# oxfordcontrol/COSMO.jl

Measured on AMD Instinct MI355X. Metric: ADMM iterations/sec (fp64) at fixed (n,m,nnz,cone), higher is better.
Workload: dtype f64

## Files before the change

cosmo.jl_amd/csrc/api.hip:

```cpp
#include <stdarg.h>
#include <stdio.h>
#include <string.h>
#include <math.h>
#include <algorithm>
#include <chrono>
#include "internal.h"
#include "device_utils.h"
#include "value_maps.h"

int32_t cosmo_fail(cosmo_hip_handle* h, int32_t code, const char* fmt, ...) {
  char buf[1024];
  va_list ap;
  va_start(ap, fmt);
  vsnprintf(buf, sizeof buf, fmt, ap);
  va_end(ap);
  if (h) h->err = buf;
  return code;
}

template <class T>
static int32_t dalloc(cosmo_hip_handle* h, T** p, size_t count) {
  if (*p) { (void)hipFree(*p); *p = nullptr; }
  if (count == 0) count = 1;
  HIPCHK(h, hipMalloc((void**)p, count * sizeof(T)));
// ... 153 lines not shown
  p->check_termination = 25; p->check_infeasibility = 40; p->adaptive_rho = 1; p->adaptive_rho_interval = 40;
  p->adaptive_rho_fraction = 0.4; p->setup_time = 0.0;
  p->unscale_residuals = 1;
  p->obj_true = (double)NAN; p->obj_true_tol = 1e-3;
}

extern "C" int32_t cosmo_hip_create(cosmo_hip_handle** out, int32_t device_id) {
  if (!out) return COSMO_HIP_ERR_INVALID;
  *out = nullptr;
  int ndev = 0;
  if (hipGetDeviceCount(&ndev) != hipSuccess || ndev <= 0) return COSMO_HIP_ERR_HIP;
  if (device_id < 0 || device_id >= ndev) return COSMO_HIP_ERR_INVALID;
  cosmo_hip_handle* h = new cosmo_hip_handle();
  h->device = device_id;
  cosmo_hip_default_params(&h->prm);
  if (hipSetDevice(device_id) != hipSuccess || hipStreamCreate(&h->stream) != hipSuccess) { delete h; return COSMO_HIP_ERR_HIP; }
  if (hipMalloc((void**)&h->ctl, sizeof(Ctl)) != hipSuccess || hipHostMalloc((void**)&h->ctl_host, sizeof(Ctl)) != hipSuccess ||
      hipMalloc((void**)&h->partials, sizeof(real) * COSMO_NSLOTS_TOTAL * COSMO_MAX_PARTIALS) != hipSuccess) {
    delete h; return COSMO_HIP_ERR_HIP;
  }
  (void)hipMemset(h->ctl, 0, sizeof(Ctl));
  (void)hipMemset(h->partials, 0, sizeof(real) * COSMO_NSLOTS_TOTAL * COSMO_MAX_PARTIALS);
  memset(h->ctl_host, 0, sizeof(Ctl));
  (void)hipEventCreate(&h->ev_proj0);
  (void)hipEventCreate(&h->ev_proj1);
  *out = h;
  return COSMO_HIP_OK;
}

static void free_vectors(cosmo_hip_handle* h) {
// ... 571 lines not shown
  CHK(h2d(h, h->ctl, h->ctl_host, 1));
  h->host_iter = 0;
  h->have_iterates = true;
  h->fb_from = h->fb_recorded;
  return COSMO_HIP_OK;
}

static const int FB_LAG = 2;
static void feedback_reset(cosmo_hip_handle* h) { h->fb_from = h->fb_recorded; }
int32_t solve_budget(cosmo_hip_handle* h, int* budget_out) {
  const int R = cosmo_hip_handle::FB_RING;
  bool& used = h->fb_used[(h->host_solves + 1) % R];
  used = false;
  if (h->fb_mode == 1 && !h->fb_k) {
    if (const char* e = getenv("COSMO_HIP_BUDGET_FEEDBACK")) { if (atoi(e) == 0) h->fb_mode = 0; }
    if (h->fb_mode == 1 && hipHostMalloc((void**)&h->fb_k, sizeof(int) * cosmo_hip_handle::FB_RING) != hipSuccess) { (void)hipGetLastError(); h->fb_k = nullptr; h->fb_mode = 0; }
  }
  *budget_out = h->budget;
  if (h->fb_mode != 1 || h->profiling || h->exact_launches) return COSMO_HIP_OK;
  const long long j = h->fb_recorded - FB_LAG;
  const int wide = h->budget + h->budget / 16;
  if (j < h->fb_from || j < 0) { *budget_out = wide > 4096 ? 4096 : wide; return COSMO_HIP_OK; }
  HIPCHK(h, hipEventSynchronize(h->fb_ev[j % R]));
  int kmax = h->fb_k[j % R], kmin = kmax, nv = 1;
  for (long long i = j - 1; i >= h->fb_from && i > j - 4; --i) { const int v = h->fb_k[i % R]; kmax = std::max(kmax, v); kmin = std::min(kmin, v); nv += 1; }
  int b = (nv >= 3) ? kmax + (kmax - kmin) / 2 + kmax / 40 + 3 : kmax + (kmax * 15 + 99) / 100 + 6;
  if (b < 3) b = 3;
  if (b > 4096) b = 4096;
  used = true;
  h->cg_k_likely = kmax + 1;
  *budget_out = b;
  return COSMO_HIP_OK;
}
int32_t feedback_record(cosmo_hip_handle* h) {
  if (h->fb_mode != 1 || !h->fb_k) return COSMO_HIP_OK;
  const int R = cosmo_hip_handle::FB_RING;
  const int slot = (int)(h->fb_recorded % R);
  if (!h->fb_ev[slot]) HIPCHK(h, hipEventCreateWithFlags(&h->fb_ev[slot], hipEventDisableTiming));
  HIPCHK(h, hipMemcpyAsync(&h->fb_k[slot], &h->ctl->cg_k, sizeof(int), hipMemcpyDeviceToHost, h->stream));
  HIPCHK(h, hipEventRecord(h->fb_ev[slot], h->stream));
  h->fb_recorded += 1;
  return COSMO_HIP_OK;
}

static int32_t enqueue_solve_in_loop(cosmo_hip_handle* h) {
  CHK(enqueue_rhs(h, 1));
  CHK(kkt_enqueue_loop_solve(h));
  h->host_solves += 1;
  return COSMO_HIP_OK;
}

static bool inf_due(const cosmo_hip_handle* h, long long it) {
  const long long ci = h->prm.check_infeasibility;
  if (ci <= 0 || ci > (1LL << 40)) return false;
// ... 478 lines not shown
```

cosmo.jl_amd/csrc/internal.h:

```cpp
#pragma once
#include <hip/hip_runtime.h>
#include <stdint.h>
#include <string>
#include <vector>
#include "../../include/cosmo_hip.h"

typedef cosmo_hip_real real;
#ifdef COSMO_HIP_REAL_FLOAT
typedef float2 real2;
#define make_real2 make_float2
#define REAL_EPS 1.1920928955078125e-07f
#define REAL_MAX 3.402823466e+38f
#define REAL_IS_FLOAT 1
#else
typedef double2 real2;
#define make_real2 make_double2
#define REAL_EPS 2.220446049250313e-16
#define REAL_MAX 1.7976931348623157e308
#define REAL_IS_FLOAT 0
#endif
#define R(x) ((real)(x))

#define COSMO_BS 256
#define COSMO_NNZ_PER_BLOCK 2048
// ... 195 lines not shown
  real *w = nullptr, *w_prev = nullptr, *s = nullptr, *mu = nullptr, *s_tl = nullptr;
  real *ls_x = nullptr, *ls_s = nullptr, *x_tl = nullptr, *nu = nullptr;
  real *rhs = nullptr, *r = nullptr, *u = nullptr, *c = nullptr, *tmp_m = nullptr, *y2 = nullptr;
  real *mr = nullptr;
  real* partials = nullptr;
  Ctl* ctl = nullptr;
  Ctl* ctl_host = nullptr;
  real* io = nullptr;
  cosmo_hip_params prm;
  long long host_iter = 0;
  long long host_solves = 0;
  int budget = 12;
  long long stalls = 0;
  static const int FB_RING = 64;
  int* fb_k = nullptr;
  hipEvent_t fb_ev[FB_RING] = {};
  long long fb_recorded = 0;
  long long fb_from = 0;
  int fb_mode = 1;
  long long fb_stalls = 0;
  bool fb_used[FB_RING] = {};
  int cg_k_likely = 0x7fffffff;
  long long spmv_calls[3] = {0, 0, 0};
  bool profiling = false;
  bool exact_launches = false;
  std::vector<hipEvent_t> ev_pool;
  std::vector<std::pair<int, int>> ev_open;
  size_t ev_used = 0;
  double kc_seconds[COSMO_HIP_NUM_KERNEL_CLASSES] = {0};
  long long kc_launches[COSMO_HIP_NUM_KERNEL_CLASSES] = {0};
// ... 24 lines not shown
    int32_t rc__ = (call);                \
    if (rc__ != COSMO_HIP_OK) return rc__; \
  } while (0)

void build_row_blocks(const std::vector<int>& rowptr, int nrows, std::vector<int>& rb, int tile_override);
int32_t upload_csr(cosmo_hip_handle* h, const HostCsr& M, CsrDev& D, int split_col, int tile_override = 0);
void free_csr(CsrDev& D);
void prof_begin(cosmo_hip_handle* h, int kc);
void prof_end(cosmo_hip_handle* h);
int32_t prof_collect(cosmo_hip_handle* h);
int32_t sync_ctl(cosmo_hip_handle* h);
int32_t rebuild_cone_plans(cosmo_hip_handle* h);
int32_t reclassify_after_scaling(cosmo_hip_handle* h);
int32_t solve_budget(cosmo_hip_handle* h, int* budget_out);
int32_t feedback_record(cosmo_hip_handle* h);

int32_t build_op_split(cosmo_hip_handle* h, bool any_a, bool fold, int factor_min, long long factor_fill_min);
int32_t refresh_op_split(cosmo_hip_handle* h);
void free_op_split(cosmo_hip_handle* h);

int32_t kkt_configure(cosmo_hip_handle* h, bool force_split);
void kkt_free(cosmo_hip_handle* h);
int32_t kkt_update_rho(cosmo_hip_handle* h);
int32_t kkt_enqueue_refresh(cosmo_hip_handle* h);
int32_t kkt_enqueue_start(cosmo_hip_handle* h, int guard, real tol_k);
int32_t kkt_enqueue_iterations(cosmo_hip_handle* h, int guard, int k_begin, int count);
int32_t kkt_enqueue_loop_solve(cosmo_hip_handle* h);
int32_t kkt_solve_now(cosmo_hip_handle* h);
int32_t kkt_resume(cosmo_hip_handle* h, int extra);
bool kkt_krylov_model(const cosmo_hip_handle* h, double* bytes, int* launches);
// ... 122 lines not shown
```

cosmo.jl_amd/csrc/kernels.hip:

```cpp
#include "device_utils.h"

__global__ __launch_bounds__(COSMO_BS) void k_spmv_plain(CsrView M, const real* __restrict__ x, real* __restrict__ y) {
  __shared__ real lds[COSMO_NNZ_PER_BLOCK];
  __shared__ real red[COSMO_BS / 64];
  for (int b = blockIdx.x; b < M.nb; b += gridDim.x) {
    csr_stream_tile(M, x, x, tile_of_block(b, M.nb, M.xcd_affine), lds, red, [&](int r, real s1, real s2) { y[r] = s1 + s2; });
  }
}

__device__ __forceinline__ real project_simple(real x, uint32_t meta, const real* __restrict__ bl,
                                                 const real* __restrict__ bu) {
  const uint32_t kind = meta & 3u;
  if (kind == 0u) return x;
  if (kind == 1u) return 0.0;
  if (kind == 2u) {
    return (x != x) ? x : ((x > R(0.0)) ? x : R(0.0));
  }
  const uint32_t j = meta >> 2;
  const real l = bl[j], u = bu[j];
  return (x < l) ? l : ((x > u) ? u : x);
}

__global__ __launch_bounds__(COSMO_BS) void k_z(const Ctl* __restrict__ ctl, int guard, long long n, long long m,
                                                const real* __restrict__ w, real* __restrict__ w_prev,
// ... 322 lines not shown
    acc += ri * ri;
  }
  acc = block_sum(acc, red);
  if constexpr (PC) accz = block_sum(accz, red);
  if (threadIdx.x == 0) {
    part_rr[blockIdx.x] = acc;
    if constexpr (PC) part_rz[blockIdx.x] = accz;
    if (blockIdx.x == 0) ctl->cg_k = k + 1;
  }
}

__global__ __launch_bounds__(COSMO_BS) void k_tail(Ctl* __restrict__ ctl, int loop_mode, CsrView A, long long n, long long m,
                                                   real alpha, const real* __restrict__ x_tl,
                                                   const real* __restrict__ ls_s, const real* __restrict__ rho,
                                                   const real* __restrict__ s, real* __restrict__ nu,
                                                   real* __restrict__ s_tl, real* __restrict__ w, int nblk_rows) {
  if (loop_mode) {
    if (ctl->halt) return;
    if (!ctl->cg_done) {
      if (blockIdx.x == 0 && threadIdx.x == 0) { ctl->stalled = 1; ctl->halt = 1; }
      return;
    }
  }
  __shared__ real lds[COSMO_NNZ_PER_BLOCK];
  __shared__ real red[COSMO_BS / 64];
  if ((int)blockIdx.x < nblk_rows) {
    for (int k = blockIdx.x; k < A.nb; k += nblk_rows) {
      csr_stream_tile(A, x_tl, x_tl, k, lds, red, [&](int row, real s1, real s2) {
        const real ax = s1 + s2;
        const real rh = rho[row];
        const real nv = (ax - ls_s[row]) * rh;
        nu[row] = nv;
        if (loop_mode) {
          const real sv = s[row];
          const real wv = w[n + row];
          const real st = (R(2.0) * sv - wv) - nv / rh;
          s_tl[row] = st;
          w[n + row] = wv + alpha * (st - sv);
        }
      });
    }
  } else if (loop_mode) {
    const long long nb2 = gridDim.x - nblk_rows;
    for (long long i = (long long)(blockIdx.x - nblk_rows) * COSMO_BS + threadIdx.x; i < n; i += nb2 * COSMO_BS) {
      const real wv = w[i];
      w[i] = wv + alpha * (x_tl[i] - wv);
    }
    if ((int)blockIdx.x == nblk_rows && threadIdx.x == 0) {
      const int k = ctl->cg_k;
      ctl->iter += 1;
      ctl->solves += 1;
      ctl->kkt_iters_total += k;
      if (k > ctl->cg_k_max) ctl->cg_k_max = k;
    }
  }
}

__global__ void k_count_solve(Ctl* __restrict__ ctl) {
  const int k = ctl->cg_k;
  ctl->solves += 1;
  ctl->kkt_iters_total += k;
  if (k > ctl->cg_k_max) ctl->cg_k_max = k;
}

__global__ __launch_bounds__(COSMO_BS) void k_chk_prim(const Ctl* __restrict__ ctl, int guard, CsrView A, long long n,
                                                       const real* __restrict__ w_prev, const real* __restrict__ s,
                                                       const real* __restrict__ b, const real* __restrict__ rho,
                                                       const real* __restrict__ Einv, real* __restrict__ mu,
// ... 383 lines not shown
  return COSMO_HIP_OK;
}

int32_t enqueue_y2_only(cosmo_hip_handle* h) {
  hipLaunchKernelGGL(k_y2_only, dim3(ew_grid(h->m > 0 ? h->m : 1)), dim3(COSMO_BS), 0, h->stream, h->ctl, h->m, h->ls_s,
                     h->rho, h->y2);
  HIPCHK(h, hipGetLastError());
  return COSMO_HIP_OK;
}

int32_t enqueue_tail(cosmo_hip_handle* h, int loop_mode) {
  const int gr = h->A.grid > 0 ? h->A.grid : 1;
  const int gx = loop_mode ? ew_grid(h->n) : 0;
  prof_begin(h, KC_TAIL);
  hipLaunchKernelGGL(k_tail, dim3(gr + gx), dim3(COSMO_BS), 0, h->stream, h->ctl, loop_mode, view_of(h->A), h->n, h->m,
                     h->prm.alpha, h->x_tl, h->ls_s, h->rho, h->s, h->nu, h->s_tl, h->w, gr);
  prof_end(h);
  h->spmv_calls[0] += 1;
  HIPCHK(h, hipGetLastError());
  return COSMO_HIP_OK;
}

int32_t enqueue_count_solve(cosmo_hip_handle* h) {
  hipLaunchKernelGGL(k_count_solve, dim3(1), dim3(1), 0, h->stream, h->ctl);
  HIPCHK(h, hipGetLastError());
  return COSMO_HIP_OK;
}

int32_t enqueue_clear_stall(cosmo_hip_handle* h) {
  hipLaunchKernelGGL(k_ctl_clear_stall, dim3(1), dim3(1), 0, h->stream, h->ctl);
  HIPCHK(h, hipGetLastError());
// ... 125 lines not shown
```

cosmo.jl_amd/csrc/polar_tiles.h:

```cpp
#pragma once
#include <algorithm>
#include <vector>

constexpr int kPolarXcds = 8;
constexpr int kPolarPanelK = 16, kPolarStreamKTile = 96;

struct PolarCone {
  int idx;
  int off, d, kind;
  int ts;
  int sk;
  int skg, skc;
  int ld;
  long long woff;
};

struct BatchCone { long long woff; int off, d, kind, ld, idx, ts; };

struct QTile { int cone, ti, tj, pad; };

struct alignas(32) RTile { int cone; int i0, j0; int ext; int ld, d; long long woff; };

struct alignas(16) RPair { int cone; int i0, j0, i1, j1; int ext0, ext1; int ld, d; int pad; long long woff; };

// ... 16 lines not shown
struct PolarBatchPlan {
  std::vector<BatchCone> cones;
  long long work = 0;
  std::vector<QTile> qtiles;
  int nbtiles = 0, nbtiles96 = 0;
  std::vector<RTile> rtiles;
  std::vector<RTile> items;
  std::vector<RPair> pairs;
  int xoff[kPolarXcds + 1] = {};
  std::vector<int> cone_nt;
  int df_ntiles = 0;
  double flops_performed = 0.0, flops_useful = 0.0;
};
const char* polar_plan_batch(const std::vector<PolarBatchIn>& in, const PolarTileOpts& o, PolarBatchPlan& out);

long long polar_tile_cost(int d, int ext);

struct LiftDepth {
  int k, streak, patience;
  bool fail(int cap) {
    const bool up = k < cap;
    if (up) k += 1;
    streak = 0;
    patience = std::min(96, 2 * patience);
    return up;
  }
  bool pass(int floor) {
    if (++streak < patience || k <= floor) return false;
    k -= 1; streak = 0;
    return true;
// ... 3 lines not shown
```

cosmo.jl_amd/csrc/psd_polar.hip:

```cpp
#include "psd_internal.h"
#include "polar_tiles.h"
#include <math.h>
#include <stdlib.h>
#include <string.h>
#include <algorithm>
#include <mutex>

#define PK 16
#ifndef POLAR_PREFETCH_DEPTH
#define POLAR_PREFETCH_DEPTH 2
#endif
#define PLD 80
static_assert(PK == kPolarPanelK, "the planner's k panel");
static_assert(sizeof(QTile) == sizeof(int4), "the quadrant list is uploaded as the kernels' int4 array");

struct SkSync { unsigned ticket; unsigned timeout; unsigned pad[14]; unsigned flag[1]; };
struct PolarDev {
  int gate;
  int rounds;
  int verified;
  int unverified;
  int projections;
  int pad[3];
  real err_last, err_max;
// ... 26 lines not shown
  PolarDev* dev = nullptr;
  PolarDev seen;
  long long launches[4] = {0, 0, 0, 0};
  int streamk = 0;
  real* sk_scratch = nullptr;
  SkSync* sk_sync = nullptr;
  int sk_gmax = 0;
  unsigned sk_base = 0, sk_epoch = 0;
  int products_last_large = 0, products_last_batch = 0;
  std::vector<BatchCone> bcones;
  BatchCone* d_bcones = nullptr;
  int4* d_btiles = nullptr;
  int nbtiles = 0, nbtiles96 = 0;
  int speculate = 0;
  int* gate_host = nullptr;
  int batch_wave = 0;
  int batch_ragged = 1;
  void* d_rtiles = nullptr;
  int nrtiles = 0;
  int dataflow = 0;
  void* d_df_tiles = nullptr;
  int* d_df_cone_nt = nullptr;
  unsigned* d_df_sync = nullptr;
  int df_xoff[9] = {0, 0, 0, 0, 0, 0, 0, 0, 0};
  int df_grid = 0;
  int df_pair = 3;
  int df_ntiles = 0;
  long long df_launches = 0, df_timed = 0;
  int df_nprod = 0;
  double df_seconds = 0.0;
// ... 1147 lines not shown
__global__ __launch_bounds__(COSMO_BS) void k_bpolar_scale(const Ctl* __restrict__ ctl, int guard, const BatchCone* __restrict__ cones,
                                                           const real* __restrict__ parts, real* __restrict__ W, real* __restrict__ bnrm,
                                                           const int* __restrict__ ubuf) {
  if (guard && ctl->halt) return;
  const BatchCone cn = cones[blockIdx.y];
  real nf2 = 0.0;
  for (int k = 0; k < BPX; ++k) nf2 += parts[(size_t)blockIdx.y * 2 * BPX + k];
  const real nf = sqrt(nf2);
  const real inv = (nf > R(0.0)) ? R(2.0) / nf : R(0.0);
  if (blockIdx.x == 0 && threadIdx.x == 0) bnrm[blockIdx.y] = nf;
  const long long n2 = (long long)cn.ld * cn.ld;
  const real* X = W + cn.woff;
  real* U = W + cn.woff + (ubuf ? ubuf[blockIdx.y] : 1) * n2;
  for (long long i = (long long)blockIdx.x * COSMO_BS + threadIdx.x; i < n2; i += (long long)gridDim.x * COSMO_BS) U[i] = X[i] * inv;
}
__global__ __launch_bounds__(COSMO_BS) void k_bpolar_finish(const Ctl* __restrict__ ctl, int guard, const BatchCone* __restrict__ cones,
                                                            real* __restrict__ W, int iu, real* __restrict__ s, real* __restrict__ parts) {
  if (guard && ctl->halt) return;
  __shared__ real red[COSMO_BS / 64];
  const BatchCone cn = cones[blockIdx.y];
  const long long n2 = (long long)cn.ld * cn.ld;
  const real* X = W + cn.woff;
  const real* U = W + cn.woff + iu * n2;
  const real* H = W + cn.woff + 3 * n2;
  real* x = s + cn.off;
  const int d = cn.d, ld = cn.ld;
  real tr = 0.0;
  for (int j = blockIdx.x; j < d; j += gridDim.x) {
    for (int i = threadIdx.x; i <= j; i += COSMO_BS) {
      const long long o = (long long)j * ld + i;
      const real v = (X[o] + H[o]) / R(2.0);
      polar_write(x, cn.kind, d, i, j, v);
      const real u = U[o];
      tr += (i == j) ? (u + u * u) : R(2.0) * u * u;
    }
  }
  tr = block_sum(tr, red);
  if (threadIdx.x == 0) parts[(size_t)blockIdx.y * 2 * BPX + BPX + blockIdx.x] = tr;
}
__global__ void k_bpolar_rank(const Ctl* __restrict__ ctl, int guard, int n, const BatchCone* __restrict__ cones, const real* __restrict__ parts,
                              int* __restrict__ rank) {
  if (guard && ctl->halt) return;
  const int c = blockIdx.x * blockDim.x + threadIdx.x;
  if (c >= n) return;
  real tr = 0.0;
  for (int k = 0; k < BPX; ++k) tr += parts[(size_t)c * 2 * BPX + BPX + k];
  rank[cones[c].idx] = (int)llround(tr / (cones[c].kind == COSMO_HIP_PSD_TRIANGLE_COMPLEX ? R(4.0) : R(2.0)));
}

__global__ __launch_bounds__(COSMO_BS) void k_bpolar_sumsq(const Ctl* __restrict__ ctl, int guard, const int* __restrict__ gate, const BatchCone* __restrict__ cones,
                                                           const real* __restrict__ W, int ig, real* __restrict__ vparts) {
  if (guard && ctl->halt) return;
  if (gate && !gate[blockIdx.y]) return;
  __shared__ real red[COSMO_BS / 64];
  const BatchCone cn = cones[blockIdx.y];
  const long long n2 = (long long)cn.ld * cn.ld;
  const real* G = W + cn.woff + ig * n2;
  real acc = 0.0;
  for (long long i = (long long)blockIdx.x * COSMO_BS + threadIdx.x; i < n2; i += (long long)gridDim.x * COSMO_BS) { const real v = G[i]; acc += v * v; }
  acc = block_sum(acc, red);
  if (threadIdx.x == 0) vparts[(size_t)blockIdx.y * BPX + blockIdx.x] = acc;
}
__global__ __launch_bounds__(COSMO_BS) void k_bpolar_decide(const Ctl* __restrict__ ctl, int guard, PolarDev* __restrict__ pd, int* __restrict__ bgate, int round,
                                                            int last, int n, const BatchCone* __restrict__ cones, const real* __restrict__ vparts,
                                                            const real* __restrict__ bnrm, real tol_factor) {
  if (guard && ctl->halt) return;
  if (round > 0 && !pd->gate) return;
  __shared__ real red[COSMO_BS / 64];
  real emax = 0.0, nfail = 0.0, nchk = 0.0;
  for (int c = threadIdx.x; c < n; c += COSMO_BS) {
    if (round > 0 && !bgate[c]) continue;
    real g2 = 0.0;
    for (int k = 0; k < BPX; ++k) g2 += vparts[(size_t)c * BPX + k];
    const real nf = bnrm[c];
    const real err = (nf > R(0.0)) ? R(0.5) * sqrt(g2) / nf : R(0.0);
    const bool ok = !(err > tol_factor * cones[c].d * PSD_EPS);
    bgate[c] = (!ok && !last) ? 1 : 0;
    nchk += 1.0;
    if (!ok) nfail += 1.0;
    emax = (err > emax || err != err) ? err : emax;
  }
  emax = block_max(emax, red);
  nfail = block_sum(nfail, red);
  nchk = block_sum(nchk, red);
  if (threadIdx.x != 0) return;
  pd->err_last = emax;
  if (emax > pd->err_max || emax != emax) pd->err_max = emax;
  if (round == 0) pd->projections += 1; else pd->rounds += 1;
  if (nfail == R(0.0)) { pd->verified += 1; pd->gate = 0; }
  else if (last) { pd->unverified += 1; pd->gate = 0; }
  else pd->gate = 1;
  (void)nchk;
}

}

void polar_plan_destroy(cosmo_hip_handle* h) {
  PolarPlan* q = static_cast<PolarPlan*>(h->psd_polar);
  if (!q) return;
  if (q->W) (void)hipFree(q->W);
  if (q->parts) (void)hipFree(q->parts);
  if (q->nrm) (void)hipFree(q->nrm);
  if (q->gate_host) (void)hipHostFree(q->gate_host);
  if (q->sk_scratch) (void)hipFree(q->sk_scratch);
  if (q->sk_sync) (void)hipFree(q->sk_sync);
  if (q->d_bcones) (void)hipFree(q->d_bcones);
  if (q->d_btiles) (void)hipFree(q->d_btiles);
  if (q->d_rtiles) (void)hipFree(q->d_rtiles);
  if (q->d_rtiles_rep) (void)hipFree(q->d_rtiles_rep);
  if (q->rep_host) (void)hipHostFree(q->rep_host);
  free(q->h_rtiles);
  if (q->BW) (void)hipFree(q->BW);
  if (q->bparts) (void)hipFree(q->bparts);
  if (q->bnrm) (void)hipFree(q->bnrm);
  if (q->bgate) (void)hipFree(q->bgate);
  if (q->d_lgate) (void)hipFree(q->d_lgate);
  if (q->d_ubuf) (void)hipFree(q->d_ubuf);
  if (q->bgate_host) (void)hipHostFree(q->bgate_host);
// ... 1 lines not shown
  if (q->d_df_cone_nt) (void)hipFree(q->d_df_cone_nt);
  if (q->d_df_sync) (void)hipFree(q->d_df_sync);
  if (q->df_ev[0]) { (void)hipEventDestroy(q->df_ev[0]); (void)hipEventDestroy(q->df_ev[1]); }
  if (q->dev) (void)hipFree(q->dev);
  delete q;
  h->psd_polar = nullptr;
}

bool polar_enabled(const cosmo_hip_handle* h) { return h->psd_polar != nullptr; }

struct PolarKnobs {
  int large_jacobi = -1, k_lift = -1, adapt = 0, compact_repair = 1, rescale = 1, speculate = -1, rounds = -1, patience = 3;
  int streamk = 0, ts = 0, sk = 0;
  long long skg = 0;
  int ts96 = 0, wave = 0, flat = 0, ragged = 1, paired = -1, sort = 1, dataflow = -1, dataflow_grid = -1, occ = -1;
};

static PolarKnobs polar_read_knobs() {
  PolarKnobs k;
  auto flag = [](const char* name, int dflt) { const char* e = getenv(name); return e ? (atoi(e) ? 1 : 0) : dflt; };
  auto within = [](const char* name, int lo, int hi, int dflt) { const char* e = getenv(name); const int v = e ? atoi(e) : dflt; return (v >= lo && v <= hi) ? v : dflt; };
  if (const char* e = getenv("COSMO_HIP_PSD_LARGE")) k.large_jacobi = (e[0] == 'j') ? 1 : 0;
  if (const char* e = getenv("COSMO_HIP_POLAR_KLIFT")) k.k_lift = std::min(40, std::max(0, atoi(e)));
  k.adapt = flag("COSMO_HIP_POLAR_ADAPT", k.adapt);
  if (const char* e = getenv("COSMO_HIP_POLAR_PATIENCE")) k.patience = std::max(1, atoi(e));
  k.compact_repair = flag("COSMO_HIP_POLAR_COMPACT_REPAIR", k.compact_repair);
  k.rescale = flag("COSMO_HIP_POLAR_RESCALE", k.rescale);
  k.speculate = flag("COSMO_HIP_POLAR_SPECULATE", k.speculate);
  if (const char* e = getenv("COSMO_HIP_POLAR_ROUNDS")) k.rounds = std::min(8, std::max(0, atoi(e)));
  k.streamk = flag("COSMO_HIP_POLAR_STREAMK", k.streamk);
  if (const char* e = getenv("COSMO_HIP_POLAR_TS")) k.ts = atoi(e);
  if (const char* e = getenv("COSMO_HIP_POLAR_SK")) k.sk = atoi(e);
  if (const char* e = getenv("COSMO_HIP_POLAR_SKG")) k.skg = atoll(e);
  k.ts96 = flag("COSMO_HIP_POLAR_BATCH_TS96", k.ts96);
  k.wave = flag("COSMO_HIP_POLAR_BATCH_WAVE", k.wave);
  k.flat = getenv("COSMO_HIP_POLAR_BATCH_FLAT") ? 1 : 0;
  k.ragged = flag("COSMO_HIP_POLAR_BATCH_RAGGED", k.ragged);
  k.sort = flag("COSMO_HIP_POLAR_BATCH_SORT", k.sort);
  k.occ = within("COSMO_HIP_POLAR_BATCH_OCC", 3, 4, k.occ);
  k.paired = within("COSMO_HIP_POLAR_PAIRED", 0, 3, k.paired);
  k.dataflow = flag("COSMO_HIP_POLAR_DATAFLOW", k.dataflow);
  k.dataflow_grid = within("COSMO_HIP_POLAR_DATAFLOW_GRID", 8, 8192, k.dataflow_grid);
  return k;
}

static void polar_set_func_attributes(const PolarPlan* q) {
  if (q->bcones.empty()) return;
  if (q->batch_ragged) {
    (void)hipFuncSetAttribute((const void*)k_polar_dataflow<4>, hipFuncAttributeMaxDynamicSharedMemorySize, GemmCfg<64>::SMEM);
    (void)hipFuncSetAttribute((const void*)k_polar_dataflow_pair<4>, hipFuncAttributeMaxDynamicSharedMemorySize, DF_PAIR_SMEM);
    (void)hipFuncSetAttribute((const void*)k_symm_gemm_batch_r<0, 3>, hipFuncAttributeMaxDynamicSharedMemorySize, GemmCfg<64>::SMEM);
    (void)hipFuncSetAttribute((const void*)k_symm_gemm_batch_r<1, 3>, hipFuncAttributeMaxDynamicSharedMemorySize, GemmCfg<64>::SMEM);
    (void)hipFuncSetAttribute((const void*)k_symm_gemm_batch_r<0, 4>, hipFuncAttributeMaxDynamicSharedMemorySize, GemmCfg<64>::SMEM);
    (void)hipFuncSetAttribute((const void*)k_symm_gemm_batch_r<1, 4>, hipFuncAttributeMaxDynamicSharedMemorySize, GemmCfg<64>::SMEM);
  }
  (void)hipFuncSetAttribute((const void*)k_symm_gemm_batch<0, 3, 64>, hipFuncAttributeMaxDynamicSharedMemorySize, GemmCfg<64>::SMEM);
  (void)hipFuncSetAttribute((const void*)k_symm_gemm_batch<1, 3, 64>, hipFuncAttributeMaxDynamicSharedMemorySize, GemmCfg<64>::SMEM);
// ... 24 lines not shown
  PolarPlan* q = new PolarPlan();
  h->psd_polar = q;
  q->klift_forced = k.k_lift >= 0;
  if (q->klift_forced) q->k_lift = k.k_lift;
  q->adapt = k.adapt; q->compact_repair = k.compact_repair; q->rescale = k.rescale; q->streamk = k.streamk;
  q->batch_ts96 = k.ts96; q->batch_wave = k.wave;
  q->speculate = k.speculate >= 0 ? k.speculate : (large_list.size() > 2 ? 1 : 0);
  if (k.rounds >= 0) q->max_rounds = k.rounds;
  q->batch_ragged = (k.ragged && !k.ts96 && !k.wave) ? 1 : 0;
  if (k.paired >= 0) q->df_pair = k.paired;
  PolarTileOpts o;
  o.ts96 = k.ts96; o.flat = k.flat; o.ragged = q->batch_ragged; o.pair = q->df_pair; o.sort = k.sort;
  o.streamk = k.streamk; o.ts = k.ts; o.sk = k.sk; o.skg = k.skg;
  HIPCHK(h, hipHostMalloc((void**)&q->gate_host, 8 * sizeof(int), hipHostMallocDefault));
  for (int i = 0; i < 8; ++i) q->gate_host[i] = 0;
  HIPCHK(h, hipMalloc((void**)&q->dev, sizeof(PolarDev)));
  HIPCHK(h, hipMemset(q->dev, 0, sizeof(PolarDev)));
  memset(&q->seen, 0, sizeof(PolarDev));
  if (!large_list.empty()) {
    long long woff = 0;
    for (int idx : large_list) {
      const PsdConeDev& c = p->cones[idx];
      PolarCone pc;
      pc.idx = idx; pc.off = c.off; pc.d = c.d; pc.kind = c.kind;
      polar_plan_large(o, pc);
      q->sk_gmax = std::max(q->sk_gmax, pc.skg);
      pc.woff = woff;
      woff += 4LL * pc.ld * pc.ld;
      q->cones.push_back(pc);
    }
// ... 100 lines not shown
    kmax = 0;
    for (int c = 0; c < n; ++c) kmax = std::max(kmax, q->bdepth[c].k);
    if (q->lgate_kmax != kmax) {
      std::vector<int> lg((size_t)std::max(kmax, 1) * n, 0), ub((size_t)n, 1);
      for (int c = 0; c < n; ++c) {
        const int t0 = kmax - q->bdepth[c].k;
        for (int t = t0; t < kmax; ++t) lg[(size_t)t * n + c] = 1;
        ub[(size_t)c] = (t0 & 1) ? 2 : 1;
      }
      HIPCHK(h, hipMemcpyAsync(q->d_lgate, lg.data(), sizeof(int) * lg.size(), hipMemcpyHostToDevice, st));
      HIPCHK(h, hipMemcpyAsync(q->d_ubuf, ub.data(), sizeof(int) * ub.size(), hipMemcpyHostToDevice, st));
      HIPCHK(h, hipStreamSynchronize(st));
      q->lgate_kmax = kmax;
    }
  }
  hipLaunchKernelGGL(k_bpolar_populate, dim3(BPX, n), dim3(COSMO_BS), 0, st, h->ctl, guard, q->d_bcones, s, q->BW, q->bparts);
  hipLaunchKernelGGL(k_bpolar_scale, dim3(BPX, n), dim3(COSMO_BS), 0, st, h->ctl, guard, q->d_bcones, q->bparts, q->BW, q->bnrm, adapt ? (const int*)q->d_ubuf : (const int*)nullptr);
  int iu = 1, iy = 2, products = 0;
  DfArgs dfa;
  bool df = q->dataflow && q->batch_ragged && q->nrtiles > 0 && !adapt && !h->profiling && 3 * (kmax + POLAR_NFIN) + 2 <= DF_MAX_PROD;
  dfa.nprod = 0;
  auto product = [&](int epi, const int* gate, int ia, int ib, int icin, int ic, real alpha, real beta) {
    if (df) { DfProd& pr = dfa.prod[dfa.nprod++]; pr.ia = ia; pr.ib = ib; pr.icin = icin; pr.ic = ic; pr.epi = epi; pr.pad = 0; pr.alpha = alpha; pr.beta = beta; return; }
    if (epi) launch_bgemm<1>(q, st, h->ctl, guard, gate, ia, ib, icin, ic, alpha, beta);
    else launch_bgemm<0>(q, st, h->ctl, guard, gate, ia, ib, icin, ic, alpha, beta);
  };
  auto flush_dataflow = [&]() -> int32_t {
    if (!df) return COSMO_HIP_OK;
    for (int x = 0; x < 9; ++x) dfa.xoff[x] = q->df_xoff[x];
    HIPCHK(h, hipMemsetAsync(q->d_df_sync, 0, sizeof(unsigned) * (DF_SYNC_DONE + q->bcones.size()), st));
    if (!q->df_ev[0]) { HIPCHK(h, hipEventCreate(&q->df_ev[0])); HIPCHK(h, hipEventCreate(&q->df_ev[1])); }
    if (q->df_ev_pending && hipEventQuery(q->df_ev[1]) == hipSuccess) {
      float ms = 0.f;
      if (hipEventElapsedTime(&ms, q->df_ev[0], q->df_ev[1]) == hipSuccess) { q->df_seconds += 1e-3 * (double)ms; q->df_timed += 1; }
      q->df_ev_pending = 0;
    }
    (void)hipGetLastError();
    const bool timed = !q->df_ev_pending;
    if (timed) HIPCHK(h, hipEventRecord(q->df_ev[0], st));
    if (q->df_pair)
      hipLaunchKernelGGL((k_polar_dataflow_pair<4>), dim3(q->df_grid), dim3(512), DF_PAIR_SMEM, st, h->ctl, guard, (const RPair*)q->d_df_tiles, (const int*)q->d_df_cone_nt,
                         q->d_df_sync, q->BW, dfa);
    else
      hipLaunchKernelGGL((k_polar_dataflow<4>), dim3(q->df_grid), dim3(256), GemmCfg<64>::SMEM, st, h->ctl, guard, (const RTile*)q->d_df_tiles, (const int*)q->d_df_cone_nt,
                         q->d_df_sync, q->BW, dfa);
// ... 3 lines not shown
    return COSMO_HIP_OK;
  };
  auto step = [&](const real* co, const int* gate) {
    product(0, gate, iu, iu, iu, iy, 1.0, 0.0);
    product(1, gate, iy, iy, iy, 3, co[2], co[1]);
    product(1, gate, iu, 3, iu, iy, 1.0, co[0]);
    std::swap(iu, iy);
    products += 3; q->launches[3] += 3;
  };
  auto verify = [&](int round, const int* gate) -> int32_t {
    product(0, gate, iu, 0, 0, 3, 1.0, 0.0);
    product(1, gate, iu, 3, 0, iy, 1.0, -1.0);
    CHK(flush_dataflow());
    hipLaunchKernelGGL(k_bpolar_sumsq, dim3(BPX, n), dim3(COSMO_BS), 0, st, h->ctl, guard, gate, q->d_bcones, q->BW, iy, vparts);
    hipLaunchKernelGGL(k_bpolar_decide, dim3(1), dim3(COSMO_BS), 0, st, h->ctl, guard, q->dev, q->bgate, round, round == q->max_rounds ? 1 : 0, n, q->d_bcones,
                       vparts, q->bnrm, q->tol_factor);
    products += 2; q->launches[3] += 2;
    return COSMO_HIP_OK;
  };
  for (int t = 0; t < kmax; ++t) step(kPolarLift, adapt ? (const int*)(q->d_lgate + (size_t)t * n) : (const int*)nullptr);
  for (int t = 0; t < POLAR_NFIN; ++t) step(kPolarFinish[t], nullptr);
  CHK(verify(0, nullptr));
  q->products_last_batch = products;
  { double wsum = 0.0, w3 = 0.0;
    for (int c = 0; c < n; ++c) { const double d3 = (double)q->bcones[c].d * q->bcones[c].d * q->bcones[c].d; w3 += d3; wsum += d3 * (3.0 * ((adapt ? q->bdepth[c].k : kmax) + POLAR_NFIN) + 2.0); }
    q->wprod_last = w3 > 0.0 ? wsum / w3 : 0.0; }
  for (int r = 1; r <= q->max_rounds; ++r) {
    if (!q->speculate) {
      HIPCHK(h, hipMemcpyAsync(q->gate_host, &q->dev->gate, (adapt && r == 1 ? 5 : 1) * sizeof(int), hipMemcpyDeviceToHost, st));
      if (r == 1 && q->bgate_host) HIPCHK(h, hipMemcpyAsync(q->bgate_host, q->bgate, sizeof(int) * (size_t)n, hipMemcpyDeviceToHost, st));
      HIPCHK(h, hipStreamSynchronize(st));
      if (adapt && r == 1 && q->gate_host[4] != q->seen_proj_batch) {
        q->seen_proj_batch = q->gate_host[4];
        q->depth_proj += 1;
        bool changed = false;
        for (int c = 0; c < n; ++c) {
          if (*q->gate_host && q->bgate_host[c]) { q->depth_fail += 1; if (q->bdepth[c].fail(POLAR_LIFT_CAP)) changed = true; }
          else if (q->bdepth[c].pass(0)) { q->depth_down += 1; changed = true; }
        }
        if (changed) q->lgate_kmax = -1;
      }
      if (!*q->gate_host) break;
// ... 4 lines not shown
        const RTile* all = (const RTile*)q->h_rtiles; RTile* dst = (RTile*)q->rep_host;
        int cnt = 0;
        for (int t = 0; t < q->nrtiles; ++t) if (all[t].cone >= 0 && q->bgate_host[all[t].cone]) dst[cnt++] = all[t];
        if (cnt > 0) {
          HIPCHK(h, hipMemcpyAsync(q->d_rtiles_rep, dst, sizeof(RTile) * (size_t)cnt, hipMemcpyHostToDevice, st));
          q->nrep = cnt; q->repair_trains += 1;
        }
        if (adapt) rlift = 1;
      }
    }
    for (int t = 0; t < rlift; ++t) step(kPolarLift, q->bgate);
    for (int t = 0; t < POLAR_NFIN; ++t) step(kPolarFinish[t], q->bgate);
    CHK(verify(r, q->bgate));
  }
  q->nrep = 0;
  hipLaunchKernelGGL(k_bpolar_finish, dim3(BPX, n), dim3(COSMO_BS), 0, st, h->ctl, guard, q->d_bcones, q->BW, iu, s, q->bparts);
  hipLaunchKernelGGL(k_bpolar_rank, dim3((n + 63) / 64), dim3(64), 0, st, h->ctl, guard, n, q->d_bcones, q->bparts, p->rank);
  HIPCHK(h, hipGetLastError());
  return COSMO_HIP_OK;
}

int32_t polar_enqueue_project(cosmo_hip_handle* h, real* s, int guard) {
  PolarPlan* q = static_cast<PolarPlan*>(h->psd_polar);
  PsdPlan* p = h->psd;
  hipStream_t st = h->stream;
  for (size_t ci = 0; ci < q->cones.size(); ++ci) {
    const PolarCone& cn = q->cones[ci];
    const long long n2 = (long long)cn.ld * cn.ld;
    real* X = q->W + cn.woff;
    real* U = X + n2;
    real* Y = U + n2;
    real* T = Y + n2;
// ... 249 lines not shown
```

Before: 377.4.

## Use mapped host memory for feedback and polar gates, speculatively launch finish kernels

```diff
diff --git a/cosmo.jl_amd/csrc/api.hip b/cosmo.jl_amd/csrc/api.hip
--- a/cosmo.jl_amd/csrc/api.hip
+++ b/cosmo.jl_amd/csrc/api.hip
@@ -191,6 +191,7 @@
   cosmo_hip_handle* h = new cosmo_hip_handle();
   h->device = device_id;
   cosmo_hip_default_params(&h->prm);
+  if (const char* e = getenv("COSMO_HIP_STEP_PASSES")) h->step_passes = atoi(e) ? 1 : 0;
   if (hipSetDevice(device_id) != hipSuccess || hipStreamCreate(&h->stream) != hipSuccess) { delete h; return COSMO_HIP_ERR_HIP; }
   if (hipMalloc((void**)&h->ctl, sizeof(Ctl)) != hipSuccess || hipHostMalloc((void**)&h->ctl_host, sizeof(Ctl)) != hipSuccess ||
       hipMalloc((void**)&h->partials, sizeof(real) * COSMO_NSLOTS_TOTAL * COSMO_MAX_PARTIALS) != hipSuccess) {
@@ -792,7 +793,12 @@
   used = false;
   if (h->fb_mode == 1 && !h->fb_k) {
     if (const char* e = getenv("COSMO_HIP_BUDGET_FEEDBACK")) { if (atoi(e) == 0) h->fb_mode = 0; }
-    if (h->fb_mode == 1 && hipHostMalloc((void**)&h->fb_k, sizeof(int) * cosmo_hip_handle::FB_RING) != hipSuccess) { (void)hipGetLastError(); h->fb_k = nullptr; h->fb_mode = 0; }
+    const bool direct = h->step_passes && !h->row_shard;
+    if (h->fb_mode == 1 && hipHostMalloc((void**)&h->fb_k, sizeof(int) * cosmo_hip_handle::FB_RING, direct ? hipHostMallocMapped | hipHostMallocCoherent : hipHostMallocDefault) != hipSuccess) { (void)hipGetLastError(); h->fb_k = nullptr; h->fb_mode = 0; }
+    if (h->fb_k && direct) {
+      for (int i = 0; i < cosmo_hip_handle::FB_RING; ++i) h->fb_k[i] = 0;
+      HIPCHK(h, hipHostGetDevicePointer((void**)&h->fb_k_dev, h->fb_k, 0));
+    }
   }
   *budget_out = h->budget;
   if (h->fb_mode != 1 || h->profiling || h->exact_launches) return COSMO_HIP_OK;
@@ -810,12 +816,16 @@
   *budget_out = b;
   return COSMO_HIP_OK;
 }
+int* feedback_slot(const cosmo_hip_handle* h) {
+  if (h->fb_mode != 1 || !h->fb_k_dev || h->row_shard || h->route == KKT_MINRES_FULL || h->route == KKT_MINRES_REDUCED) return nullptr;
+  return h->fb_k_dev + h->fb_recorded % cosmo_hip_handle::FB_RING;
+}
 int32_t feedback_record(cosmo_hip_handle* h) {
   if (h->fb_mode != 1 || !h->fb_k) return COSMO_HIP_OK;
   const int R = cosmo_hip_handle::FB_RING;
   const int slot = (int)(h->fb_recorded % R);
   if (!h->fb_ev[slot]) HIPCHK(h, hipEventCreateWithFlags(&h->fb_ev[slot], hipEventDisableTiming));
-  HIPCHK(h, hipMemcpyAsync(&h->fb_k[slot], &h->ctl->cg_k, sizeof(int), hipMemcpyDeviceToHost, h->stream));
+  if (!feedback_slot(h)) HIPCHK(h, hipMemcpyAsync(&h->fb_k[slot], &h->ctl->cg_k, sizeof(int), hipMemcpyDeviceToHost, h->stream));
   HIPCHK(h, hipEventRecord(h->fb_ev[slot], h->stream));
   h->fb_recorded += 1;
   return COSMO_HIP_OK;
diff --git a/cosmo.jl_amd/csrc/internal.h b/cosmo.jl_amd/csrc/internal.h
--- a/cosmo.jl_amd/csrc/internal.h
+++ b/cosmo.jl_amd/csrc/internal.h
@@ -233,6 +233,8 @@
   long long stalls = 0;
   static const int FB_RING = 64;
   int* fb_k = nullptr;
+  int* fb_k_dev = nullptr;
+  int step_passes = 1;
   hipEvent_t fb_ev[FB_RING] = {};
   long long fb_recorded = 0;
   long long fb_from = 0;
@@ -287,6 +289,7 @@
 int32_t reclassify_after_scaling(cosmo_hip_handle* h);
 int32_t solve_budget(cosmo_hip_handle* h, int* budget_out);
 int32_t feedback_record(cosmo_hip_handle* h);
+int* feedback_slot(const cosmo_hip_handle* h);
 
 int32_t build_op_split(cosmo_hip_handle* h, bool any_a, bool fold, int factor_min, long long factor_fill_min);
 int32_t refresh_op_split(cosmo_hip_handle* h);
diff --git a/cosmo.jl_amd/csrc/kernels.hip b/cosmo.jl_amd/csrc/kernels.hip
--- a/cosmo.jl_amd/csrc/kernels.hip
+++ b/cosmo.jl_amd/csrc/kernels.hip
@@ -360,11 +360,15 @@
                                                    real alpha, const real* __restrict__ x_tl,
                                                    const real* __restrict__ ls_s, const real* __restrict__ rho,
                                                    const real* __restrict__ s, real* __restrict__ nu,
-                                                   real* __restrict__ s_tl, real* __restrict__ w, int nblk_rows) {
+                                                   real* __restrict__ s_tl, real* __restrict__ w, int nblk_rows,
+                                                   int* __restrict__ fb_slot, int keep_s_tl) {
   if (loop_mode) {
-    if (ctl->halt) return;
-    if (!ctl->cg_done) {
-      if (blockIdx.x == 0 && threadIdx.x == 0) { ctl->stalled = 1; ctl->halt = 1; }
+    const int halt = ctl->halt;
+    if (halt || !ctl->cg_done) {
+      if (blockIdx.x == 0 && threadIdx.x == 0) {
+        if (fb_slot) *fb_slot = ctl->cg_k;
+        if (!halt) { ctl->stalled = 1; ctl->halt = 1; }
+      }
       return;
     }
   }
@@ -381,7 +385,7 @@
           const real sv = s[row];
           const real wv = w[n + row];
           const real st = (R(2.0) * sv - wv) - nv / rh;
-          s_tl[row] = st;
+          if (keep_s_tl) s_tl[row] = st;
           w[n + row] = wv + alpha * (st - sv);
         }
       });
@@ -398,6 +402,7 @@
       ctl->solves += 1;
       ctl->kkt_iters_total += k;
       if (k > ctl->cg_k_max) ctl->cg_k_max = k;
+      if (fb_slot) *fb_slot = k;
     }
   }
 }
@@ -811,7 +816,8 @@
   const int gx = loop_mode ? ew_grid(h->n) : 0;
   prof_begin(h, KC_TAIL);
   hipLaunchKernelGGL(k_tail, dim3(gr + gx), dim3(COSMO_BS), 0, h->stream, h->ctl, loop_mode, view_of(h->A), h->n, h->m,
-                     h->prm.alpha, h->x_tl, h->ls_s, h->rho, h->s, h->nu, h->s_tl, h->w, gr);
+                     h->prm.alpha, h->x_tl, h->ls_s, h->rho, h->s, h->nu, h->s_tl, h->w, gr, loop_mode ? feedback_slot(h) : (int*)nullptr,
+                     (loop_mode && h->step_passes) ? 0 : 1);
   prof_end(h);
   h->spmv_calls[0] += 1;
   HIPCHK(h, hipGetLastError());
diff --git a/cosmo.jl_amd/csrc/polar_tiles.h b/cosmo.jl_amd/csrc/polar_tiles.h
--- a/cosmo.jl_amd/csrc/polar_tiles.h
+++ b/cosmo.jl_amd/csrc/polar_tiles.h
@@ -54,6 +54,15 @@
 };
 const char* polar_plan_batch(const std::vector<PolarBatchIn>& in, const PolarTileOpts& o, PolarBatchPlan& out);
 
+struct PolarWg { int cone, bx; };
+constexpr int polar_wg_grid(int n, int bpx) { return kPolarXcds * bpx * ((n + kPolarXcds - 1) / kPolarXcds); }
+constexpr int polar_wg_id(int cone, int bx, int bpx) { return kPolarXcds * ((cone / kPolarXcds) * bpx + bx) + cone % kPolarXcds; }
+constexpr PolarWg polar_wg_decode(int id, int n, int bpx) {
+  const int xcd = id & (kPolarXcds - 1), slot = id / kPolarXcds;
+  const int cone = kPolarXcds * (slot / bpx) + xcd;
+  return (id < 0 || cone >= n) ? PolarWg{-1, 0} : PolarWg{cone, slot % bpx};
+}
+
 long long polar_tile_cost(int d, int ext);
 
 struct LiftDepth {
diff --git a/cosmo.jl_amd/csrc/psd_polar.hip b/cosmo.jl_amd/csrc/psd_polar.hip
--- a/cosmo.jl_amd/csrc/psd_polar.hip
+++ b/cosmo.jl_amd/csrc/psd_polar.hip
@@ -64,6 +64,10 @@
   int nbtiles = 0, nbtiles96 = 0;
   int speculate = 0;
   int* gate_host = nullptr;
+  int step_passes = 1;
+  int* gate_map = nullptr;
+  int* gate_map_dev = nullptr;
+  hipEvent_t gate_ev = nullptr;
   int batch_wave = 0;
   int batch_ragged = 1;
   void* d_rtiles = nullptr;
@@ -1241,9 +1245,54 @@
   real* U = W + cn.woff + (ubuf ? ubuf[blockIdx.y] : 1) * n2;
   for (long long i = (long long)blockIdx.x * COSMO_BS + threadIdx.x; i < n2; i += (long long)gridDim.x * COSMO_BS) U[i] = X[i] * inv;
 }
-__global__ __launch_bounds__(COSMO_BS) void k_bpolar_finish(const Ctl* __restrict__ ctl, int guard, const BatchCone* __restrict__ cones,
+__global__ __launch_bounds__(COSMO_BS) void k_bpolar_norm(const Ctl* __restrict__ ctl, int guard, int n, const BatchCone* __restrict__ cones,
+                                                          const real* __restrict__ s, real* __restrict__ parts) {
+  if (guard && ctl->halt) return;
+  const PolarWg wg = polar_wg_decode((int)blockIdx.x, n, BPX);
+  if (wg.cone < 0) return;
+  __shared__ real red[COSMO_BS / 64];
+  const BatchCone cn = cones[wg.cone];
+  const real* x = s + cn.off;
+  const int d = cn.d;
+  real acc = 0.0;
+  for (int j = wg.bx; j < d; j += BPX) {
+    for (int i = threadIdx.x; i < d; i += COSMO_BS) { const real v = polar_read(x, cn.kind, d, i, j); acc += v * v; }
+  }
+  acc = block_sum(acc, red);
+  if (threadIdx.x == 0) parts[(size_t)wg.cone * 2 * BPX + wg.bx] = acc;
+}
+__global__ __launch_bounds__(COSMO_BS) void k_bpolar_populate2(const Ctl* __restrict__ ctl, int guard, int n, const BatchCone* __restrict__ cones,
+                                                               const real* __restrict__ s, const real* __restrict__ parts, real* __restrict__ W,
+                                                               real* __restrict__ bnrm, const int* __restrict__ ubuf, unsigned* __restrict__ sync, int nsync) {
+  if (guard && ctl->halt) return;
+  if (sync && blockIdx.x == 0) for (int k = threadIdx.x; k < nsync; k += COSMO_BS) sync[k] = 0u;
+  const PolarWg wg = polar_wg_decode((int)blockIdx.x, n, BPX);
+  if (wg.cone < 0) return;
+  const BatchCone cn = cones[wg.cone];
+  real nf2 = 0.0;
+  for (int k = 0; k < BPX; ++k) nf2 += parts[(size_t)wg.cone * 2 * BPX + k];
+  const real nf = sqrt(nf2);
+  const real inv = (nf > R(0.0)) ? R(2.0) / nf : R(0.0);
+  if (wg.bx == 0 && threadIdx.x == 0) bnrm[wg.cone] = nf;
+  const real* x = s + cn.off;
+  const int d = cn.d, ld = cn.ld;
+  real* X = W + cn.woff;
+  real* U = X + (ubuf ? ubuf[wg.cone] : 1) * (long long)ld * ld;
+  for (int j = wg.bx; j < ld; j += BPX) {
+    for (int i = threadIdx.x; i < ld; i += COSMO_BS) {
+      real v = 0.0;
+      if (i < d && j < d) v = polar_read(x, cn.kind, d, i, j);
+      const long long o = (long long)j * ld + i;
+      X[o] = v;
+      U[o] = v * inv;
+    }
+  }
+}
+__global__ __launch_bounds__(COSMO_BS) void k_bpolar_finish(const Ctl* __restrict__ ctl, int guard, const int* __restrict__ skip_if,
+                                                            const BatchCone* __restrict__ cones,
                                                             real* __restrict__ W, int iu, real* __restrict__ s, real* __restrict__ parts) {
   if (guard && ctl->halt) return;
+  if (skip_if && *skip_if) return;
   __shared__ real red[COSMO_BS / 64];
   const BatchCone cn = cones[blockIdx.y];
   const long long n2 = (long long)cn.ld * cn.ld;
@@ -1265,9 +1314,10 @@
   tr = block_sum(tr, red);
   if (threadIdx.x == 0) parts[(size_t)blockIdx.y * 2 * BPX + BPX + blockIdx.x] = tr;
 }
-__global__ void k_bpolar_rank(const Ctl* __restrict__ ctl, int guard, int n, const BatchCone* __restrict__ cones, const real* __restrict__ parts,
-                              int* __restrict__ rank) {
+__global__ void k_bpolar_rank(const Ctl* __restrict__ ctl, int guard, const int* __restrict__ skip_if, int n, const BatchCone* __restrict__ cones,
+                              const real* __restrict__ parts, int* __restrict__ rank) {
   if (guard && ctl->halt) return;
+  if (skip_if && *skip_if) return;
   const int c = blockIdx.x * blockDim.x + threadIdx.x;
   if (c >= n) return;
   real tr = 0.0;
@@ -1290,7 +1340,7 @@
 }
 __global__ __launch_bounds__(COSMO_BS) void k_bpolar_decide(const Ctl* __restrict__ ctl, int guard, PolarDev* __restrict__ pd, int* __restrict__ bgate, int round,
                                                             int last, int n, const BatchCone* __restrict__ cones, const real* __restrict__ vparts,
-                                                            const real* __restrict__ bnrm, real tol_factor) {
+                                                            const real* __restrict__ bnrm, real tol_factor, int* __restrict__ gate_map) {
   if (guard && ctl->halt) return;
   if (round > 0 && !pd->gate) return;
   __shared__ real red[COSMO_BS / 64];
@@ -1314,9 +1364,12 @@
   pd->err_last = emax;
   if (emax > pd->err_max || emax != emax) pd->err_max = emax;
   if (round == 0) pd->projections += 1; else pd->rounds += 1;
-  if (nfail == R(0.0)) { pd->verified += 1; pd->gate = 0; }
-  else if (last) { pd->unverified += 1; pd->gate = 0; }
-  else pd->gate = 1;
+  int g = 0;
+  if (nfail == R(0.0)) pd->verified += 1;
+  else if (last) pd->unverified += 1;
+  else g = 1;
+  pd->gate = g;
+  if (gate_map) *gate_map = g;
   (void)nchk;
 }
 
@@ -1329,6 +1382,8 @@
   if (q->parts) (void)hipFree(q->parts);
   if (q->nrm) (void)hipFree(q->nrm);
   if (q->gate_host) (void)hipHostFree(q->gate_host);
+  if (q->gate_map) (void)hipHostFree(q->gate_map);
+  if (q->gate_ev) (void)hipEventDestroy(q->gate_ev);
   if (q->sk_scratch) (void)hipFree(q->sk_scratch);
   if (q->sk_sync) (void)hipFree(q->sk_sync);
   if (q->d_bcones) (void)hipFree(q->d_bcones);
@@ -1360,6 +1415,7 @@
   int streamk = 0, ts = 0, sk = 0;
   long long skg = 0;
   int ts96 = 0, wave = 0, flat = 0, ragged = 1, paired = -1, sort = 1, dataflow = -1, dataflow_grid = -1, occ = -1;
+  int step_passes = 1;
 };
 
 static PolarKnobs polar_read_knobs() {
@@ -1387,6 +1443,7 @@
   k.paired = within("COSMO_HIP_POLAR_PAIRED", 0, 3, k.paired);
   k.dataflow = flag("COSMO_HIP_POLAR_DATAFLOW", k.dataflow);
   k.dataflow_grid = within("COSMO_HIP_POLAR_DATAFLOW_GRID", 8, 8192, k.dataflow_grid);
+  k.step_passes = flag("COSMO_HIP_STEP_PASSES", k.step_passes);
   return k;
 }
 
@@ -1441,6 +1498,13 @@
   o.streamk = k.streamk; o.ts = k.ts; o.sk = k.sk; o.skg = k.skg;
   HIPCHK(h, hipHostMalloc((void**)&q->gate_host, 8 * sizeof(int), hipHostMallocDefault));
   for (int i = 0; i < 8; ++i) q->gate_host[i] = 0;
+  q->step_passes = k.step_passes;
+  if (q->step_passes) {
+    HIPCHK(h, hipHostMalloc((void**)&q->gate_map, 16 * sizeof(int), hipHostMallocMapped | hipHostMallocCoherent));
+    for (int i = 0; i < 16; ++i) q->gate_map[i] = 0;
+    HIPCHK(h, hipHostGetDevicePointer((void**)&q->gate_map_dev, q->gate_map, 0));
+    HIPCHK(h, hipEventCreateWithFlags(&q->gate_ev, hipEventDisableTiming));
+  }
   HIPCHK(h, hipMalloc((void**)&q->dev, sizeof(PolarDev)));
   HIPCHK(h, hipMemset(q->dev, 0, sizeof(PolarDev)));
   memset(&q->seen, 0, sizeof(PolarDev));
@@ -1571,11 +1635,19 @@
       q->lgate_kmax = kmax;
     }
   }
-  hipLaunchKernelGGL(k_bpolar_populate, dim3(BPX, n), dim3(COSMO_BS), 0, st, h->ctl, guard, q->d_bcones, s, q->BW, q->bparts);
-  hipLaunchKernelGGL(k_bpolar_scale, dim3(BPX, n), dim3(COSMO_BS), 0, st, h->ctl, guard, q->d_bcones, q->bparts, q->BW, q->bnrm, adapt ? (const int*)q->d_ubuf : (const int*)nullptr);
-  int iu = 1, iy = 2, products = 0;
   DfArgs dfa;
   bool df = q->dataflow && q->batch_ragged && q->nrtiles > 0 && !adapt && !h->profiling && 3 * (kmax + POLAR_NFIN) + 2 <= DF_MAX_PROD;
+  const bool df_cleared = df && q->step_passes;
+  if (q->step_passes) {
+    const int grid = polar_wg_grid(n, BPX);
+    hipLaunchKernelGGL(k_bpolar_norm, dim3(grid), dim3(COSMO_BS), 0, st, h->ctl, guard, n, q->d_bcones, s, q->bparts);
+    hipLaunchKernelGGL(k_bpolar_populate2, dim3(grid), dim3(COSMO_BS), 0, st, h->ctl, guard, n, q->d_bcones, s, q->bparts, q->BW, q->bnrm,
+                       adapt ? (const int*)q->d_ubuf : (const int*)nullptr, df_cleared ? q->d_df_sync : (unsigned*)nullptr, DF_SYNC_DONE + n);
+  } else {
+    hipLaunchKernelGGL(k_bpolar_populate, dim3(BPX, n), dim3(COSMO_BS), 0, st, h->ctl, guard, q->d_bcones, s, q->BW, q->bparts);
+    hipLaunchKernelGGL(k_bpolar_scale, dim3(BPX, n), dim3(COSMO_BS), 0, st, h->ctl, guard, q->d_bcones, q->bparts, q->BW, q->bnrm, adapt ? (const int*)q->d_ubuf : (const int*)nullptr);
+  }
+  int iu = 1, iy = 2, products = 0;
   dfa.nprod = 0;
   auto product = [&](int epi, const int* gate, int ia, int ib, int icin, int ic, real alpha, real beta) {
     if (df) { DfProd& pr = dfa.prod[dfa.nprod++]; pr.ia = ia; pr.ib = ib; pr.icin = icin; pr.ic = ic; pr.epi = epi; pr.pad = 0; pr.alpha = alpha; pr.beta = beta; return; }
@@ -1585,7 +1657,7 @@
   auto flush_dataflow = [&]() -> int32_t {
     if (!df) return COSMO_HIP_OK;
     for (int x = 0; x < 9; ++x) dfa.xoff[x] = q->df_xoff[x];
-    HIPCHK(h, hipMemsetAsync(q->d_df_sync, 0, sizeof(unsigned) * (DF_SYNC_DONE + q->bcones.size()), st));
+    if (!df_cleared) HIPCHK(h, hipMemsetAsync(q->d_df_sync, 0, sizeof(unsigned) * (DF_SYNC_DONE + q->bcones.size()), st));
     if (!q->df_ev[0]) { HIPCHK(h, hipEventCreate(&q->df_ev[0])); HIPCHK(h, hipEventCreate(&q->df_ev[1])); }
     if (q->df_ev_pending && hipEventQuery(q->df_ev[1]) == hipSuccess) {
       float ms = 0.f;
@@ -1619,7 +1691,7 @@
     CHK(flush_dataflow());
     hipLaunchKernelGGL(k_bpolar_sumsq, dim3(BPX, n), dim3(COSMO_BS), 0, st, h->ctl, guard, gate, q->d_bcones, q->BW, iy, vparts);
     hipLaunchKernelGGL(k_bpolar_decide, dim3(1), dim3(COSMO_BS), 0, st, h->ctl, guard, q->dev, q->bgate, round, round == q->max_rounds ? 1 : 0, n, q->d_bcones,
-                       vparts, q->bnrm, q->tol_factor);
+                       vparts, q->bnrm, q->tol_factor, q->gate_map_dev);
     products += 2; q->launches[3] += 2;
     return COSMO_HIP_OK;
   };
@@ -1630,7 +1702,15 @@
   { double wsum = 0.0, w3 = 0.0;
     for (int c = 0; c < n; ++c) { const double d3 = (double)q->bcones[c].d * q->bcones[c].d * q->bcones[c].d; w3 += d3; wsum += d3 * (3.0 * ((adapt ? q->bdepth[c].k : kmax) + POLAR_NFIN) + 2.0); }
     q->wprod_last = w3 > 0.0 ? wsum / w3 : 0.0; }
-  for (int r = 1; r <= q->max_rounds; ++r) {
+  bool finished = false;
+  if (q->step_passes && !adapt && !q->speculate && !h->profiling && q->max_rounds >= 1) {
+    HIPCHK(h, hipEventRecord(q->gate_ev, st));
+    hipLaunchKernelGGL(k_bpolar_finish, dim3(BPX, n), dim3(COSMO_BS), 0, st, h->ctl, guard, (const int*)&q->dev->gate, q->d_bcones, q->BW, iu, s, q->bparts);
+    hipLaunchKernelGGL(k_bpolar_rank, dim3((n + 63) / 64), dim3(64), 0, st, h->ctl, guard, (const int*)&q->dev->gate, n, q->d_bcones, q->bparts, p->rank);
+    HIPCHK(h, hipEventSynchronize(q->gate_ev));
+    finished = *(volatile int*)q->gate_map == 0;
+  }
+  for (int r = 1; r <= q->max_rounds && !finished; ++r) {
     if (!q->speculate) {
       HIPCHK(h, hipMemcpyAsync(q->gate_host, &q->dev->gate, (adapt && r == 1 ? 5 : 1) * sizeof(int), hipMemcpyDeviceToHost, st));
       if (r == 1 && q->bgate_host) HIPCHK(h, hipMemcpyAsync(q->bgate_host, q->bgate, sizeof(int) * (size_t)n, hipMemcpyDeviceToHost, st));
@@ -1665,8 +1745,10 @@
     CHK(verify(r, q->bgate));
   }
   q->nrep = 0;
-  hipLaunchKernelGGL(k_bpolar_finish, dim3(BPX, n), dim3(COSMO_BS), 0, st, h->ctl, guard, q->d_bcones, q->BW, iu, s, q->bparts);
-  hipLaunchKernelGGL(k_bpolar_rank, dim3((n + 63) / 64), dim3(64), 0, st, h->ctl, guard, n, q->d_bcones, q->bparts, p->rank);
+  if (!finished) {
+    hipLaunchKernelGGL(k_bpolar_finish, dim3(BPX, n), dim3(COSMO_BS), 0, st, h->ctl, guard, (const int*)nullptr, q->d_bcones, q->BW, iu, s, q->bparts);
+    hipLaunchKernelGGL(k_bpolar_rank, dim3((n + 63) / 64), dim3(64), 0, st, h->ctl, guard, (const int*)nullptr, n, q->d_bcones, q->bparts, p->rank);
+  }
   HIPCHK(h, hipGetLastError());
   return COSMO_HIP_OK;
 }
```

Result: faster. 382.3 (median of 6 runs) (+1.3%).
